# imazen/codec-eval

Measured on AMD Instinct MI355X. Metric: metric MP/s (SSIMULACRA2+DSSIM+Butteraugli) at 1/2/4/8 GPU; HBM-roofline %, higher is better.
Workload: dtype f32

## Files before the change

codec-eval_amd/csrc/dssim.hip:

```cpp
#include <algorithm>
#include <cstdlib>

#include "ce_internal.h"
#include "dssim_common.h"

namespace {

constexpr int TPB = 256;

__device__ __forceinline__ uint32_t slot_of(uint32_t z, uint32_t n_refs_used, uint32_t max_refs)
{
    return z < n_refs_used ? z : max_refs + (z - n_refs_used);
}

__global__ __launch_bounds__(TPB) void k_rgb8_to_rgba_f32(const uint8_t *__restrict__ rgb, const float *__restrict__ lut,
                                                          float4 *__restrict__ out, size_t n)
{
    __shared__ float s_lut[256];
    s_lut[threadIdx.x] = lut[threadIdx.x];
    __syncthreads();
    for (size_t i = (size_t)blockIdx.x * TPB + threadIdx.x; i < n; i += (size_t)gridDim.x * TPB)
        out[i] = make_float4(s_lut[rgb[3 * i]], s_lut[rgb[3 * i + 1]], s_lut[rgb[3 * i + 2]], 1.0f);
}

__device__ __forceinline__ double block_sum(double v, double *s_red)
{
#pragma unroll
    for (int off = 32; off > 0; off >>= 1) v += __shfl_down(v, off, 64);
    if ((threadIdx.x & 63) == 0) s_red[threadIdx.x >> 6] = v;
    __syncthreads();
    double t = 0.0;
    if (threadIdx.x == 0)
        for (int k = 0; k < TPB / 64; k++) t += s_red[k];
    __syncthreads();
    return t;
}

struct ds_tail {
    uint32_t w[CE_DSSIM_SCALES], h[CE_DSSIM_SCALES], pitch[CE_DSSIM_SCALES], n_part[CE_DSSIM_SCALES], gx[CE_DSSIM_SCALES];
    uint32_t blk_end[CE_DSSIM_SCALES];
    size_t plane[CE_DSSIM_SCALES], map_off[CE_DSSIM_SCALES];
};

__global__ __launch_bounds__(TPB) void k_dssim_avg(const double *__restrict__ part, double *__restrict__ avg_out, ds_tail t, uint32_t n_levels,
                                                   uint32_t n_blocks)
{
    __shared__ double s_red[TPB];
    const uint32_t p = blockIdx.x, level = blockIdx.y;
    const double *pp = part + ((size_t)p * n_levels + level) * 2 * n_blocks;
    const uint32_t used_blocks = t.n_part[level];
    double v = 0.0;
    for (uint32_t k = threadIdx.x; k < used_blocks; k += TPB) v += pp[k];
    s_red[threadIdx.x] = v;
    __syncthreads();
    for (int off = TPB / 2; off > 0; off >>= 1) {
        if ((int)threadIdx.x < off) s_red[threadIdx.x] += s_red[threadIdx.x + off];
        __syncthreads();
    }
    if (threadIdx.x == 0) {
        double avg = s_red[0] / (double)((size_t)t.w[level] * t.h[level]);
        if (!(avg > 0.0)) avg = 0.0;
        avg_out[(size_t)p * n_levels + level] = pow(avg, pow(0.5, (double)level));
    }
}

constexpr int AD_ROWS = 32;
__global__ __launch_bounds__(TPB) void k_dssim_absdev(const float *__restrict__ map, const double *__restrict__ avg_in,
                                                      double *__restrict__ part, ds_tail t, uint32_t n_levels, uint32_t n_blocks)
{
    __shared__ double s_red[TPB / 64];
    const uint32_t per_pair = t.blk_end[n_levels - 1], p = blockIdx.x / per_pair, bi = blockIdx.x % per_pair;
    uint32_t level = 0, first = 0;
#pragma unroll
    for (int l = 0; l + 1 < CE_DSSIM_SCALES; l++)
        if (l + 1 < (int)n_levels && bi >= t.blk_end[l]) level = l + 1, first = t.blk_end[l];
    const uint32_t w = t.w[level], h = t.h[level], pitch = t.pitch[level], gx = t.gx[level];
    const uint32_t bx = (bi - first) % gx, by = (bi - first) / gx;
    double *pp = part + ((size_t)p * n_levels + level) * 2 * n_blocks;
    const double avg = avg_in[(size_t)p * n_levels + level];
    const float *m = map + t.map_off[level] + (size_t)p * t.plane[level];
    const uint32_t x = bx * 64 + (threadIdx.x & 63);
    double val = 0.0;
#pragma unroll
    for (int k = 0; k < AD_ROWS / 4; k++) {
        const uint32_t y = by * AD_ROWS + 4 * k + (threadIdx.x >> 6);
        if (x < w && y < h) val += fabs(avg - (double)m[(size_t)y * pitch + x]);
    }
    const double s = block_sum(val, s_red);
    if (threadIdx.x == 0) pp[n_blocks + by * gx + bx] = s;
}

struct ds_geom {
    uint32_t npix[CE_DSSIM_SCALES];
    uint32_t nblk[CE_DSSIM_SCALES];
};

__global__ __launch_bounds__(64) void k_dssim_finalize_pairs(const double *__restrict__ part, double *__restrict__ level_scores,
                                                             ce_dev_scores *__restrict__ scores, uint32_t n_pairs,
                                                             uint32_t n_levels, uint32_t n_blocks, ds_geom g)
{
    const uint32_t p = blockIdx.x, lane = threadIdx.x;
    if (p >= n_pairs) return;
    const double W[CE_DSSIM_SCALES] = {0.028, 0.197, 0.322, 0.298, 0.155};
    double ssim_sum = 0.0, weight_sum = 0.0;
    for (uint32_t l = 0; l < n_levels; l++) {
        const double *pp = part + (((size_t)p * n_levels + l) * 2 + 1) * n_blocks;
        double dev = 0.0;
        for (uint32_t k = lane; k < g.nblk[l]; k += 64) dev += pp[k];
#pragma unroll
        for (int off = 32; off > 0; off >>= 1) dev += __shfl_down(dev, off, 64);
        dev = __shfl(dev, 0, 64);
        const double score = 1.0 - dev / (double)g.npix[l];
        if (lane == 0) level_scores[(size_t)p * CE_DSSIM_SCALES + l] = score;
        ssim_sum += score * W[l];
        weight_sum += W[l];
    }
    double ssim = ssim_sum / weight_sum;
    if (!(ssim > 2.220446049250313e-16)) ssim = 2.220446049250313e-16;
    if (lane == 0) scores[p].dssim = 1.0 / ssim - 1.0;
}

size_t map_offset(const ce_batch *b, int l)
{
    size_t off = 0;
    for (int k = 0; k < l; k++) off += (size_t)b->max_pairs * b->ds[k].plane;
    return off;
}

}

void ce_dssim_free(ce_batch *b)
{
    for (auto &p : b->ds_lin) hipFree(p), p = nullptr;
    hipFree(b->ds_img); hipFree(b->ds_map);
    for (int l = 0; l < CE_DSSIM_SCALES; l++) {
        hipFree(b->ds_rimg[l]); hipFree(b->ds_rmu[l]); hipFree(b->ds_rsq[l]);
        b->ds_rimg[l] = b->ds_rmu[l] = b->ds_rsq[l] = nullptr;
        ce_free_xcd_list(&b->ds_gwork[l]);
    }
    b->ds_ref_src = nullptr;
    hipFree(b->ds_part); hipFree(b->ds_level_scores); hipFree(b->ds_cells);
    b->ds_img = b->ds_map = b->ds_cells = nullptr;
    b->ds_cells_cap = 0;
    b->ds_map_pairs = 0;
    b->ds_part = b->ds_level_scores = nullptr;
    b->dssim_ready = false;
}

static int dssim_allocate(ce_batch *b)
{
    ce_ctx *ctx = b->ctx;
    uint32_t lw[CE_DSSIM_SCALES], lh[CE_DSSIM_SCALES];
    const int n = (int)ce_plan_dssim_levels(b->w, b->h, CE_DSSIM_SCALES, lw, lh);
    for (int l = 0; l < n; l++) {
        auto &d = b->ds[l];
        d.w = lw[l];
        d.h = lh[l];
        d.pitch = (d.w + 31u) & ~31u;
        d.plane = (size_t)d.pitch * d.h;
    }
    b->ds_levels = n;
    const size_t slots = (size_t)b->max_refs + b->max_pairs, p0 = b->ds[0].plane;
    const size_t p1 = n > 1 ? b->ds[1].plane : 1;
    CE_HIP(ctx, hipMalloc(&b->ds_lin[0], slots * 3 * p1 * sizeof(float)));
    CE_HIP(ctx, hipMalloc(&b->ds_lin[1], slots * 3 * p1 * sizeof(float)));
    CE_HIP(ctx, hipMalloc(&b->ds_img, (size_t)b->max_pairs * 3 * p0 * sizeof(float)));
    for (int l = 0; l < n; l++) {
        const size_t rb = (size_t)b->max_refs * 3 * b->ds[l].plane * sizeof(float);
        CE_HIP(ctx, hipMalloc(&b->ds_rimg[l], rb));
        CE_HIP(ctx, hipMalloc(&b->ds_rmu[l], rb));
        CE_HIP(ctx, hipMalloc(&b->ds_rsq[l], rb));
    }
    CE_HIP(ctx, hipMalloc(&b->ds_map, map_offset(b, n) * sizeof(float)));
    b->ds_blocks = std::max(((b->ds[0].w + 63) / 64) * ((b->ds[0].h + AD_ROWS - 1) / AD_ROWS), ((b->ds[0].w + CE_DSSIM_STRIP - 1) / CE_DSSIM_STRIP) * ((b->ds[0].h + 1) / 2));
    CE_HIP(ctx, hipMalloc(&b->ds_part, (size_t)b->max_pairs * CE_DSSIM_SCALES * 2 * b->ds_blocks * sizeof(double)));
    CE_HIP(ctx, hipMalloc(&b->ds_level_scores, (size_t)b->max_pairs * CE_DSSIM_SCALES * sizeof(double)));
    return CE_OK;
}

static int dssim_prepare(ce_batch *b)
{
    if (b->dssim_ready) return CE_OK;
    const int rc = dssim_allocate(b);
    if (rc != CE_OK) {
        const std::string why = b->ctx->err;
        ce_dssim_free(b);
        (void)hipGetLastError();
        b->ctx->err = why;
        return rc;
    }
    b->dssim_ready = true;
    return CE_OK;
}

int ce_launch_dssim(ce_batch *b, const uint8_t *d_refs, uint32_t n_refs_used, uint32_t n_pairs)
{
    ce_ctx *ctx = b->ctx;
    int rc = dssim_prepare(b);
    if (rc != CE_OK) return rc;
    const bool cached = b->keep_ref_pyramid && b->ds_ref_src == d_refs && b->ds_ref_count >= n_refs_used;
    const uint32_t z0 = cached ? n_refs_used : 0;
    if (!cached) b->ref_builds[1]++;
    ds_geom g{};
    ds_tail tail{};
    for (int l = 0; l < b->ds_levels; l++) {
        const auto &d = b->ds[l];
        if ((rc = ce_dssim_create_stream(b, l, d_refs, n_refs_used, n_pairs, z0)) != CE_OK) return rc;
        uint32_t n_part = 0;
        if ((rc = ce_dssim_compare_stream(b, l, n_pairs, b->ds_map + map_offset(b, l), &n_part)) != CE_OK) return rc;
        tail.w[l] = d.w, tail.h[l] = d.h, tail.pitch[l] = d.pitch, tail.plane[l] = d.plane, tail.n_part[l] = n_part;
        tail.gx[l] = (d.w + 63) / 64;
        tail.map_off[l] = map_offset(b, l);
        g.npix[l] = d.w * d.h;
        g.nblk[l] = tail.gx[l] * ((d.h + AD_ROWS - 1) / AD_ROWS);
        tail.blk_end[l] = (l ? tail.blk_end[l - 1] : 0u) + g.nblk[l];
    }
    {
        const uint32_t nl = (uint32_t)b->ds_levels;
        CE_LAUNCH(ctx, "dssim_avg", k_dssim_avg, dim3(n_pairs, nl), dim3(TPB), 0, b->ds_part, b->ds_level_scores, tail, nl, b->ds_blocks);
        const dim3 gp(tail.blk_end[nl - 1] * n_pairs);
        CE_LAUNCH(ctx, "dssim_absdev", k_dssim_absdev, gp, dim3(TPB), 0, (const float *)b->ds_map, b->ds_level_scores, b->ds_part, tail, nl,
                  b->ds_blocks);
    }
    if (b->keep_ref_pyramid && !cached) {
        b->ds_ref_src = d_refs;
        b->ds_ref_count = n_refs_used;
    }
    CE_LAUNCH(ctx, "dssim_finalize", k_dssim_finalize_pairs, dim3(n_pairs), dim3(64), 0, b->ds_part,
              b->ds_level_scores, b->d_scores, n_pairs, (uint32_t)b->ds_levels, b->ds_blocks, g);
    CE_HIP(ctx, hipGetLastError());
    return CE_OK;
}

int ce_dssim_read_maps(ce_batch *b, uint32_t level, uint32_t first, uint32_t count, uint32_t block, float *maps, double *ssim)
{
    ce_ctx *ctx = b->ctx;
    if (ssim) {
        CE_HIP(ctx, hipMemcpy2DAsync(ssim, sizeof(double), b->ds_level_scores + (size_t)first * CE_DSSIM_SCALES + level,
                                     CE_DSSIM_SCALES * sizeof(double), sizeof(double), count, hipMemcpyDeviceToHost, ctx->stream));
        if (!maps) CE_HIP(ctx, hipStreamSynchronize(ctx->stream));
    }
    if (!maps) return CE_OK;
    const auto &d = b->ds[level];
    return ce_read_map_cells(b, "dssim_block_min", b->ds_map + map_offset(b, (int)level), ce_map_geom{d.w, d.h, d.pitch, d.plane},
                             first, count, block, true, &b->ds_cells, &b->ds_cells_cap, maps);
}

int ce_launch_rgb8_to_dssim_image(ce_ctx *ctx, const uint8_t *d_rgb, float *d_rgba, size_t n_pixels)
{
    if (n_pixels == 0) return CE_OK;
    size_t blocks = std::min<size_t>((n_pixels + TPB - 1) / TPB, 4096);
    CE_LAUNCH(ctx, "rgb8_to_dssim_image", k_rgb8_to_rgba_f32, dim3((uint32_t)blocks), dim3(TPB), 0, d_rgb, ctx->d_lut_powf,
              reinterpret_cast<float4 *>(d_rgba), n_pixels);
    CE_HIP(ctx, hipGetLastError());
    return CE_OK;
}
```

codec-eval_amd/csrc/dssim_stream.hip:

```cpp
#include <algorithm>
#include <cstdlib>
#include <string>
#include <type_traits>

#include "ce_internal.h"
#include "dssim_common.h"

namespace {

constexpr int CS_OUT = CE_DSSIM_STRIP;
constexpr int CS_WAVES = 4;

__device__ __forceinline__ float lane_left(float v)
{
    return __builtin_bit_cast(float, __builtin_amdgcn_mov_dpp(__builtin_bit_cast(int, v), 0x138, 0xf, 0xf, true));
}
__device__ __forceinline__ float lane_right(float v)
{
    return __builtin_bit_cast(float, __builtin_amdgcn_mov_dpp(__builtin_bit_cast(int, v), 0x130, 0xf, 0xf, true));
}
__device__ __forceinline__ float ld_at(const float *base, uint32_t byte_off)
{
    return *reinterpret_cast<const float *>(reinterpret_cast<const char *>(base) + byte_off);
}

template <int N>
struct rowsN {
    float c[N], e[N], lr[N];
};
typedef rowsN<9> rows9;
struct rowin {
    float a[3], r[3];
};

template <int NP>
__device__ __forceinline__ float pass_rows(const rowsN<NP> &P, const rowsN<NP> &M, rowsN<NP> &N, int k, float v, float c_above)
{
    const float K0 = 0.095332f, K1 = 0.118095f, K4 = 0.146293f;
    const float corners = (P.lr[k] + lane_left(v)) + lane_right(v);
    const float edges = M.e[k] + v;
    N.c[k] = v;
    N.e[k] = (c_above + lane_left(v)) + lane_right(v);
    N.lr[k] = lane_left(v) + lane_right(v);
    return corners * K0 + edges * K1 + M.c[k] * K4;
}

struct cmp_planes {
    const float *t[3], *r[3], *u[3], *q[3];
};

template <bool EDGE>
__device__ __forceinline__ double dssim_compare_strip(const cmp_planes &pl, float *__restrict__ map, const lvl_geom &g, int xs, int y0, int y1)
{
    const int w = (int)g.w, h = (int)g.h, lane = (int)(threadIdx.x & 63);
    const uint32_t pitch = g.pitch;
    const int X = xs + lane - 2;
    const uint32_t Xc = (uint32_t)min(max(X, 0), w - 1);
    const bool out_lane = lane >= 2 && lane < 2 + CS_OUT && X < w;
    const bool before_first = X == -1, after_last = X == w;
    auto row_off = [&](int y) { return ((uint32_t)min(max(y, 0), h - 1) * pitch + Xc) * 4u; };
    double val = 0.0;
    auto step = [&](auto ends, const rows9 &P1, rows9 &M1, rows9 &N1, const rows9 &P2, rows9 &M2, rows9 &N2, const rowin &cur, rowin &nxt, int i)
                    __attribute__((always_inline)) {
        constexpr bool ENDS = decltype(ends)::value;
        const int t = i - 1, y = i - 2;
        float u1[3], q1[3];
        {
            const uint32_t o = row_off(i + 1), os = row_off(y);
#pragma unroll
            for (int c = 0; c < 3; c++) {
                nxt.a[c] = ld_at(pl.t[c], o);
                nxt.r[c] = ld_at(pl.r[c], o);
                u1[c] = ld_at(pl.u[c], os);
                q1[c] = ld_at(pl.q[c], os);
            }
        }
        float O[9];
#pragma unroll
        for (int c = 0; c < 3; c++) {
            const float v3[3] = {cur.a[c], cur.r[c] * cur.a[c], cur.a[c] * cur.a[c]};
#pragma unroll
            for (int j = 0; j < 3; j++) {
                const int k = 3 * c + j;
                float T = pass_rows(P1, M1, N1, k, v3[j], M1.c[k]);
                if (EDGE) {
                    const float fl = lane_right(T), fr = lane_left(T);
                    T = before_first ? fl : (after_last ? fr : T);
                }
                float c_above = M2.c[k];
                if (ENDS && t == h) T = M2.c[k];
                if (ENDS && t == 0) c_above = T;
                O[k] = pass_rows(P2, M2, N2, k, T, c_above);
                if (ENDS && t == 0) M2.lr[k] = N2.lr[k];
            }
            __builtin_amdgcn_sched_barrier(0);
        }
        if (y >= y0 && y < y1) {
            const float c1 = 0.01f * 0.01f, c2 = 0.03f * 0.03f, third = 1.0f / 3.0f;
            float m11[3], m12[3], m22[3], s1[3], s2[3], s12c[3];
#pragma unroll
            for (int c = 0; c < 3; c++) {
                const float u2v = O[3 * c + 0], s12 = O[3 * c + 1], q2 = O[3 * c + 2];
                m11[c] = u1[c] * u1[c];
                m12[c] = u1[c] * u2v;
                m22[c] = u2v * u2v;
                s1[c] = q1[c] - m11[c];
                s2[c] = q2 - m22[c];
                s12c[c] = s12 - m12[c];
            }
#define AVG3(v) (((v)[0] + (v)[1] + (v)[2]) * third)
            const float mu1_sq = AVG3(m11), mu2_sq = AVG3(m22), mu1_mu2 = AVG3(m12);
            const float sigma1_sq = AVG3(s1), sigma2_sq = AVG3(s2), sigma12 = AVG3(s12c);
#undef AVG3
            const float ssim = (2.0f * mu1_mu2 + c1) * (2.0f * sigma12 + c2) / ((mu1_sq + mu2_sq + c1) * (sigma1_sq + sigma2_sq + c2));
            if (out_lane) {
                map[(uint32_t)y * pitch + (uint32_t)X] = ssim;
                val += (double)ssim;
            }
        }
        __builtin_amdgcn_sched_barrier(0);
    };
    rows9 s0, s1, s2, z0, z1, z2;
#pragma unroll
    for (int k = 0; k < 9; k++) s0.lr[k] = s1.c[k] = s1.e[k] = s1.lr[k] = z0.lr[k] = z1.c[k] = z1.e[k] = z1.lr[k] = 0.f;
    rowin L0, L1, L2;
    const int i0 = y0 == 0 ? -1 : y0 - 2, n_bodies = (y1 + 1 - i0) / 3 + 1;
    {
        const uint32_t o = row_off(i0);
#pragma unroll
        for (int c = 0; c < 3; c++) L0.a[c] = ld_at(pl.t[c], o), L0.r[c] = ld_at(pl.r[c], o);
    }
    auto body = [&](auto ends, int i) __attribute__((always_inline)) {
        step(ends, s0, s1, s2, z0, z1, z2, L0, L1, i);
        step(ends, s1, s2, s0, z1, z2, z0, L1, L2, i + 1);
        step(ends, s2, s0, s1, z2, z0, z1, L2, L0, i + 2);
    };
    int i = i0;
    body(std::true_type{}, i);
    i += 3;
#pragma unroll 1
    for (int b = 1; b < n_bodies - 1; b++, i += 3) body(std::false_type{}, i);
    if (n_bodies > 1) body(std::true_type{}, i);
    return val;
}

__global__ __launch_bounds__(CS_WAVES * 64) __attribute__((amdgpu_waves_per_eu(3, 3))) void k_dssim_compare_stream(const float *__restrict__ img, const float *__restrict__ rimg,
                                                                        const float *__restrict__ rmu, const float *__restrict__ rsq,
                                                                        const uint32_t *__restrict__ pair_ref, float *__restrict__ map,
                                                                        double *__restrict__ part, lvl_geom g, uint32_t level,
                                                                        uint32_t n_levels, uint32_t n_blocks,
                                                                        const uint2 *__restrict__ work, uint32_t strips, uint32_t rows)
{
    const uint32_t wv = __builtin_amdgcn_readfirstlane(threadIdx.x >> 6);
    const uint2 wi = work[((blockIdx.x >> 3) * CS_WAVES + wv) * 8 + (blockIdx.x & 7)];
    const uint32_t tile = __builtin_amdgcn_readfirstlane(wi.x), p = __builtin_amdgcn_readfirstlane(wi.y);
    if (tile == ~0u) return;
    const uint32_t ref = __builtin_amdgcn_readfirstlane(pair_ref[p]);
    const int xs = (int)(tile % strips) * CS_OUT, y0 = (int)((tile / strips) * rows), y1 = min(y0 + (int)rows, (int)g.h);
    cmp_planes pl;
#pragma unroll
    for (int c = 0; c < 3; c++) {
        pl.t[c] = img + ((size_t)p * 3 + c) * g.plane;
        pl.r[c] = rimg + ((size_t)ref * 3 + c) * g.plane;
        pl.u[c] = rmu + ((size_t)ref * 3 + c) * g.plane;
        pl.q[c] = rsq + ((size_t)ref * 3 + c) * g.plane;
    }
    float *pmap = map + (size_t)p * g.plane;
    double val = (xs == 0 || xs + CS_OUT + 2 >= (int)g.w) ? dssim_compare_strip<true>(pl, pmap, g, xs, y0, y1)
                                                          : dssim_compare_strip<false>(pl, pmap, g, xs, y0, y1);
#pragma unroll
    for (int off = 32; off > 0; off >>= 1) val += __shfl_down(val, off, 64);
    if ((threadIdx.x & 63) == 0) part[(((size_t)p * n_levels + level) * 2 + 0) * n_blocks + tile] = val;
}

constexpr int CR_HALO_REF = 4, CR_HALO_DIST = 2;

template <int SRC, bool REF, bool EDGE>
__device__ __forceinline__ void dssim_create_strip(const uint8_t *__restrict__ src8, const float *const (&srcf)[3], const float *s_lut,
                                                   float *const (&lin_out)[3], float *const (&oimg)[3], float *const (&omu)[3],
                                                   float *const (&osq)[3], const lvl_geom &g, const lvl_geom &gn, int has_next, int xs,
                                                   int y0, int y1)
{
    constexpr bool FROM_U8 = SRC == CE_SRC_U8, FROM_U16 = SRC == CE_SRC_U16;
    constexpr int H = REF ? CR_HALO_REF : CR_HALO_DIST, OUT = 64 - 2 * H;
    const int w = (int)g.w, h = (int)g.h, lane = (int)(threadIdx.x & 63);
    const uint32_t pitch = g.pitch;
    const int X = xs + lane - H;
    const uint32_t Xc = (uint32_t)min(max(X, 0), w - 1);
    const bool out_lane = lane >= H && lane < H + OUT && X < w;
    const bool before_first = X == -1, after_last = X == w;
    auto edge_fix = [&](float T) {
        if (!EDGE) return T;
        const float fl = lane_right(T), fr = lane_left(T);
        return before_first ? fl : (after_last ? fr : T);
    };
    struct rgb { float v[3]; };
    struct raw3 { uint32_t v[3]; };
    auto request = [&](int y, raw3 &o) {
        const uint32_t yc = (uint32_t)min(max(y, 0), h - 1);
        if (FROM_U8) {
            const uint8_t *px = src8 + (yc * (uint32_t)w + Xc) * 3u;
            o.v[0] = px[0], o.v[1] = px[1], o.v[2] = px[2];
        } else if (FROM_U16) {
            const uint16_t *px = reinterpret_cast<const uint16_t *>(src8) + (yc * (uint32_t)w + Xc) * 3u;
            o.v[0] = px[0], o.v[1] = px[1], o.v[2] = px[2];
        } else if (SRC == CE_SRC_LIN) {
            const float *px = reinterpret_cast<const float *>(src8) + (yc * (uint32_t)w + Xc) * 3u;
#pragma unroll
            for (int c = 0; c < 3; c++) o.v[c] = __float_as_uint(px[c]);
        } else {
            const uint32_t ob = (yc * pitch + Xc) * 4u;
#pragma unroll
            for (int c = 0; c < 3; c++) o.v[c] = __float_as_uint(ld_at(srcf[c], ob));
        }
    };
    auto linear = [&](const raw3 &r, rgb &o) {
#pragma unroll
        for (int c = 0; c < 3; c++) o.v[c] = (FROM_U8 || FROM_U16) ? s_lut[r.v[c]] : __uint_as_float(r.v[c]);
    };
    constexpr int NS = REF ? 6 : 1;
    auto later_pass = [&](auto ends, auto &P, auto &M, auto &N, int k, float v, int r) __attribute__((always_inline)) {
        constexpr bool ENDS = decltype(ends)::value;
        float c_above = M.c[k];
        if (ENDS && r == h) v = M.c[k];
        if (ENDS && r == 0) c_above = v;
        const float o = pass_rows(P, M, N, k, v, c_above);
        if (ENDS && r == 0) M.lr[k] = N.lr[k];
        return o;
    };
    auto step = [&](auto ends, const rowsN<2> &Pa, rowsN<2> &Ma, rowsN<2> &Na, const rowsN<2> &Pb, rowsN<2> &Mb, rowsN<2> &Nb,
                    const rowsN<NS> &Pm, rowsN<NS> &Mm, rowsN<NS> &Nm, const rowsN<NS> &Pq, rowsN<NS> &Mq, rowsN<NS> &Nq,
                    const rgb &cur, rgb &nxt, const rgb &prev, const raw3 &arrived, raw3 &requested, float &L_new, const float &L_out,
                    int i) __attribute__((always_inline)) {
        request(i + 2, requested);
        linear(arrived, nxt);
        if (has_next && (i & 1) && i >= y0 && i < y1) {
            const int oy = i >> 1;
            float q[3];
#pragma unroll
            for (int c = 0; c < 3; c++) q[c] = (((prev.v[c] + lane_right(prev.v[c])) + cur.v[c]) + lane_right(cur.v[c])) * 0.25f;
            if (out_lane && !(X & 1) && (X >> 1) < (int)gn.w && oy < (int)gn.h) {
                const uint32_t o = (uint32_t)oy * gn.pitch + (uint32_t)(X >> 1);
#pragma unroll
                for (int c = 0; c < 3; c++) lin_out[c][o] = q[c];
            }
        }
        float L, A, B;
        rgb_to_lab(cur.v[0], cur.v[1], cur.v[2], L, A, B);
        L_new = L;
        const float ab[2] = {A, B};
        float img[3];
        img[0] = L_out;
#pragma unroll
        for (int k = 0; k < 2; k++) {
            const float T = edge_fix(pass_rows(Pa, Ma, Na, k, ab[k], Ma.c[k]));
            img[1 + k] = later_pass(ends, Pb, Mb, Nb, k, T, i - 1);
        }
        __builtin_amdgcn_sched_barrier(0);
        const int j = i - 2;
        if (j >= y0 && j < y1 && out_lane) {
            const uint32_t o = (uint32_t)j * pitch + (uint32_t)X;
#pragma unroll
            for (int c = 0; c < 3; c++) oimg[c][o] = img[c];
        }
        if (REF) {
            float O[6];
#pragma unroll
            for (int c = 0; c < 3; c++) {
                const float v = c == 0 ? img[0] : edge_fix(img[c]);
                const float two[2] = {v, v * v};
#pragma unroll
                for (int t = 0; t < 2; t++) {
                    const int k = 2 * c + t;
                    const float T = edge_fix(later_pass(ends, Pm, Mm, Nm, k, two[t], j));
                    O[k] = later_pass(ends, Pq, Mq, Nq, k, T, j - 1);
                }
                __builtin_amdgcn_sched_barrier(0);
            }
            const int y = i - 4;
            if (y >= y0 && y < y1 && out_lane) {
                const uint32_t o = (uint32_t)y * pitch + (uint32_t)X;
#pragma unroll
                for (int c = 0; c < 3; c++) omu[c][o] = O[2 * c], osq[c][o] = O[2 * c + 1];
            }
        }
    };
    rowsN<2> a0, a1, a2, b0, b1, b2;
    rowsN<NS> m0, m1, m2, q0, q1, q2;
#pragma unroll
    for (int k = 0; k < 2; k++) a0.lr[k] = a1.c[k] = a1.e[k] = a1.lr[k] = b0.lr[k] = b1.c[k] = b1.e[k] = b1.lr[k] = 0.f;
#pragma unroll
    for (int k = 0; k < NS; k++) m0.lr[k] = m1.c[k] = m1.e[k] = m1.lr[k] = q0.lr[k] = q1.c[k] = q1.e[k] = q1.lr[k] = 0.f;
    rgb R0, R1, R2;
    float l0 = 0.f, l1 = 0.f, l2 = 0.f;
    const int i0 = y0 == 0 ? -1 : y0 - H, i_last = y1 + H - 1, n_bodies = (i_last - i0) / 3 + 1;
    raw3 W0, W1, W2;
    request(i0, W2);
    request(i0 + 1, W0);
    linear(W2, R0);
    R2 = R0;
    auto body = [&](auto ends, int i) __attribute__((always_inline)) {
        step(ends, a0, a1, a2, b0, b1, b2, m0, m1, m2, q0, q1, q2, R0, R1, R2, W0, W1, l0, l1, i);
        step(ends, a1, a2, a0, b1, b2, b0, m1, m2, m0, q1, q2, q0, R1, R2, R0, W1, W2, l1, l2, i + 1);
        step(ends, a2, a0, a1, b2, b0, b1, m2, m0, m1, q2, q0, q1, R2, R0, R1, W2, W0, l2, l0, i + 2);
    };
    int i = i0, b = 0;
#pragma unroll 1
    for (; b < min(2, n_bodies); b++, i += 3) body(std::true_type{}, i);
#pragma unroll 1
    for (; b < n_bodies - 2; b++, i += 3) body(std::false_type{}, i);
#pragma unroll 1
    for (; b < n_bodies; b++, i += 3) body(std::true_type{}, i);
}

template <int SRC>
__global__ __launch_bounds__(CS_WAVES * 64) void k_dssim_create_stream(const uint8_t *__restrict__ refs, const uint8_t *__restrict__ tests,
                                                                       const float *__restrict__ lut, const float *__restrict__ lut_test,
                                                                       const float *__restrict__ lin_in,
                                                                       float *__restrict__ lin_out, float *__restrict__ img,
                                                                       float *__restrict__ rimg, float *__restrict__ rmu,
                                                                       float *__restrict__ rsq, lvl_geom g, lvl_geom gn, int has_next,
                                                                       size_t img_bytes, uint32_t n_refs_used, uint32_t max_refs, uint32_t z0,
                                                                       uint32_t rows)
{
    constexpr bool FROM_U8 = SRC == CE_SRC_U8, FROM_U16 = SRC == CE_SRC_U16;
    __shared__ float s_lut[256];
    if (FROM_U8) {
        s_lut[threadIdx.x] = lut[threadIdx.x];
        __syncthreads();
    }
    const uint32_t wv = __builtin_amdgcn_readfirstlane(threadIdx.x >> 6);
    const uint32_t z = blockIdx.y + z0;
    const bool is_ref = z < n_refs_used;
    const uint32_t slot = is_ref ? z : max_refs + (z - n_refs_used), oslot = is_ref ? z : z - n_refs_used;
    const uint32_t out_cols = 64 - 2 * (is_ref ? CR_HALO_REF : CR_HALO_DIST), strips = (g.w + out_cols - 1) / out_cols;
    const uint32_t tile = blockIdx.x * CS_WAVES + wv;
    if (tile >= strips * ((g.h + rows - 1) / rows)) return;
    const int xs = (int)((tile % strips) * out_cols), y0 = (int)((tile / strips) * rows), y1 = min(y0 + (int)rows, (int)g.h);
    const uint8_t *src8 = (FROM_U8 || FROM_U16 || SRC == CE_SRC_LIN) ? (is_ref ? refs + (size_t)z * img_bytes : tests + (size_t)(z - n_refs_used) * img_bytes) : nullptr;
    const float *srcf[3];
    float *lo[3], *oi[3], *om[3], *oq[3];
#pragma unroll
    for (int c = 0; c < 3; c++) {
        srcf[c] = lin_in + ((size_t)slot * 3 + c) * g.plane;
        lo[c] = lin_out + ((size_t)slot * 3 + c) * gn.plane;
        oi[c] = (is_ref ? rimg : img) + ((size_t)oslot * 3 + c) * g.plane;
        om[c] = rmu + ((size_t)oslot * 3 + c) * g.plane;
        oq[c] = rsq + ((size_t)oslot * 3 + c) * g.plane;
    }
    const float *tab = FROM_U16 ? (is_ref ? lut : lut_test) : s_lut;
    const bool edge = xs == 0 || xs + (int)out_cols + (is_ref ? CR_HALO_REF : CR_HALO_DIST) >= (int)g.w;
    if (is_ref) {
        if (edge)
            dssim_create_strip<SRC, true, true>(src8, srcf, tab, lo, oi, om, oq, g, gn, has_next, xs, y0, y1);
        else
            dssim_create_strip<SRC, true, false>(src8, srcf, tab, lo, oi, om, oq, g, gn, has_next, xs, y0, y1);
    } else {
        if (edge)
            dssim_create_strip<SRC, false, true>(src8, srcf, tab, lo, oi, om, oq, g, gn, has_next, xs, y0, y1);
        else
            dssim_create_strip<SRC, false, false>(src8, srcf, tab, lo, oi, om, oq, g, gn, has_next, xs, y0, y1);
    }
}

uint32_t stream_rows(uint32_t strips, uint32_t h, uint32_t n_images)
{
    static const size_t min_waves = [] {
        const char *e = std::getenv("CE_STREAM_MIN_WAVES");
        return e ? (size_t)std::atol(e) : (size_t)8192;
    }();
    uint32_t rows = 64;
    while (rows > 8 && (size_t)strips * ((h + rows - 1) / rows) * n_images < min_waves) rows /= 2;
    while (rows > 2 && (size_t)strips * ((h + rows - 1) / rows) * n_images < 1024) rows /= 2;
    return rows;
}

}

int ce_dssim_create_stream(ce_batch *b, int l, const uint8_t *d_refs, uint32_t n_refs_used, uint32_t n_pairs, uint32_t z0)
{
    ce_ctx *ctx = b->ctx;
    const auto &d = b->ds[l];
    const bool has_next = l + 1 < b->ds_levels;
    const auto &nd = b->ds[has_next ? l + 1 : l];
    const lvl_geom lg{d.w, d.h, d.pitch, d.plane}, ng{nd.w, nd.h, nd.pitch, nd.plane};
    const uint32_t n_slots = n_refs_used + n_pairs;
    if (n_slots <= z0) return CE_OK;
    const uint32_t strips_ref = (d.w + 64 - 2 * CR_HALO_REF - 1) / (64 - 2 * CR_HALO_REF), strips = (d.w + CS_OUT - 1) / CS_OUT;
    const uint32_t rows = b->debug_ds_rows ? b->debug_ds_rows : stream_rows(strips, d.h, n_slots - z0);
    const uint32_t tiles = std::max(z0 < n_refs_used ? strips_ref : 0u, strips) * ((d.h + rows - 1) / rows);
#define CE_CREATE_LAUNCH(NAME, U8, GRID, Z0, LUT_R, LUT_T)                                                                                      \
    CE_LAUNCH(ctx, NAME, (k_dssim_create_stream<U8>), GRID, dim3(CS_WAVES * 64), 0, d_refs, (const uint8_t *)b->d_tests,            \
              (const float *)LUT_R, (const float *)LUT_T, (const float *)(l == 0 ? nullptr : b->ds_lin[l & 1]), b->ds_lin[(l + 1) & 1], b->ds_img,      \
              b->ds_rimg[l], b->ds_rmu[l], b->ds_rsq[l], lg, ng, has_next ? 1 : 0, b->img_bytes, n_refs_used, b->max_refs, Z0, rows)
    const dim3 grid((tiles + CS_WAVES - 1) / CS_WAVES, n_slots - z0);
    if (l == 0 && b->linear) CE_CREATE_LAUNCH("dssim_create_lin", CE_SRC_LIN, grid, z0, nullptr, nullptr);
    else if (l == 0 && b->depth[0]) CE_CREATE_LAUNCH("dssim_create_u16", CE_SRC_U16, grid, z0, b->deep_lut[1][0], b->deep_lut[1][1]);
    else if (l == 0) CE_CREATE_LAUNCH("dssim_create_u8", CE_SRC_U8, grid, z0, ctx->d_lut_powf, ctx->d_lut_powf);
    else CE_CREATE_LAUNCH("dssim_create", CE_SRC_F32, grid, z0, ctx->d_lut_powf, ctx->d_lut_powf);
#undef CE_CREATE_LAUNCH
    return CE_OK;
}

int ce_dssim_compare_stream(ce_batch *b, int l, uint32_t n_pairs, float *level_map, uint32_t *n_part)
{
    ce_ctx *ctx = b->ctx;
    const auto &d = b->ds[l];
    const lvl_geom lg{d.w, d.h, d.pitch, d.plane};
    const uint32_t strips = (d.w + CS_OUT - 1) / CS_OUT, rows = b->debug_ds_rows ? b->debug_ds_rows : stream_rows(strips, d.h, n_pairs);
    const int rc = ce_build_xcd_list(b, n_pairs, ce_xcd_keys{1, (d.h + rows - 1) / rows, strips, CS_WAVES}, &b->ds_gwork[l]);
    if (rc != CE_OK) return rc;
    CE_LAUNCH(ctx, "dssim_compare", k_dssim_compare_stream, dim3(b->ds_gwork[l].len / CS_WAVES), dim3(CS_WAVES * 64), 0,
              (const float *)b->ds_img, (const float *)b->ds_rimg[l], (const float *)b->ds_rmu[l], (const float *)b->ds_rsq[l],
              b->d_pair_ref, level_map, b->ds_part, lg, (uint32_t)l, (uint32_t)b->ds_levels, b->ds_blocks,
              (const uint2 *)b->ds_gwork[l].d, strips, rows);
    *n_part = strips * ((d.h + rows - 1) / rows);
    return CE_OK;
}
```

Before: 19100.

## Batch DSSIM absdev rows per block and use bpermute for edge reflection

The absdev kernel now has each block cover several consecutive 32-row tiles, prefetching the next tile's map values while it reduces the current one. This cuts the number of blocks launched and overlaps load latency with the reduction. In the streaming compare and create kernels, the two DPP moves plus selects used for edge mirroring become a single ds_bpermute with a per-lane source index. The pass_rows shuffles are hoisted, and an asm barrier pins the evaluation order of the sums. bpermute goes through the LDS crossbar, so it may add latency compared with DPP. The extra per-block serial loop also reduces parallelism on the smaller pyramid levels.

Measured after the change: 19320 (median of 6 runs). 1.01x the previous value.

```diff
diff --git a/codec-eval_amd/csrc/dssim.hip b/codec-eval_amd/csrc/dssim.hip
--- a/codec-eval_amd/csrc/dssim.hip
+++ b/codec-eval_amd/csrc/dssim.hip
@@ -65,6 +65,7 @@
 }
 
 constexpr int AD_ROWS = 32;
+constexpr int AD_SUB = 4;
 __global__ __launch_bounds__(TPB) void k_dssim_absdev(const float *__restrict__ map, const double *__restrict__ avg_in,
                                                       double *__restrict__ part, ds_tail t, uint32_t n_levels, uint32_t n_blocks)
 {
@@ -75,19 +76,35 @@
     for (int l = 0; l + 1 < CE_DSSIM_SCALES; l++)
         if (l + 1 < (int)n_levels && bi >= t.blk_end[l]) level = l + 1, first = t.blk_end[l];
     const uint32_t w = t.w[level], h = t.h[level], pitch = t.pitch[level], gx = t.gx[level];
-    const uint32_t bx = (bi - first) % gx, by = (bi - first) / gx;
+    const uint32_t bx = (bi - first) % gx, by0 = (bi - first) / gx * AD_SUB, by1 = min(by0 + AD_SUB, (h + AD_ROWS - 1) / AD_ROWS);
     double *pp = part + ((size_t)p * n_levels + level) * 2 * n_blocks;
     const double avg = avg_in[(size_t)p * n_levels + level];
     const float *m = map + t.map_off[level] + (size_t)p * t.plane[level];
     const uint32_t x = bx * 64 + (threadIdx.x & 63);
-    double val = 0.0;
-#pragma unroll
-    for (int k = 0; k < AD_ROWS / 4; k++) {
-        const uint32_t y = by * AD_ROWS + 4 * k + (threadIdx.x >> 6);
-        if (x < w && y < h) val += fabs(avg - (double)m[(size_t)y * pitch + x]);
-    }
-    const double s = block_sum(val, s_red);
-    if (threadIdx.x == 0) pp[n_blocks + by * gx + bx] = s;
+    float v[AD_ROWS / 4], nv[AD_ROWS / 4];
+    auto load = [&](uint32_t by, float (&o)[AD_ROWS / 4]) {
+#pragma unroll
+        for (int k = 0; k < AD_ROWS / 4; k++) {
+            const uint32_t y = by * AD_ROWS + 4 * k + (threadIdx.x >> 6);
+            o[k] = (x < w && y < h) ? m[(size_t)y * pitch + x] : 0.f;
+        }
+    };
+    load(by0, v);
+    for (uint32_t by = by0; by < by1; by++) {
+        if (by + 1 < by1) load(by + 1, nv);
+        double val = 0.0;
+#pragma unroll
+        for (int k = 0; k < AD_ROWS / 4; k++) {
+            const uint32_t y = by * AD_ROWS + 4 * k + (threadIdx.x >> 6);
+            if (x < w && y < h) val += fabs(avg - (double)v[k]);
+        }
+        const double s = block_sum(val, s_red);
+        if (threadIdx.x == 0) pp[n_blocks + by * gx + bx] = s;
+        if (by + 1 < by1) {
+#pragma unroll
+            for (int k = 0; k < AD_ROWS / 4; k++) v[k] = nv[k];
+        }
+    }
 }
 
 struct ds_geom {
@@ -213,7 +230,7 @@
         tail.map_off[l] = map_offset(b, l);
         g.npix[l] = d.w * d.h;
         g.nblk[l] = tail.gx[l] * ((d.h + AD_ROWS - 1) / AD_ROWS);
-        tail.blk_end[l] = (l ? tail.blk_end[l - 1] : 0u) + g.nblk[l];
+        tail.blk_end[l] = (l ? tail.blk_end[l - 1] : 0u) + tail.gx[l] * (((d.h + AD_ROWS - 1) / AD_ROWS + AD_SUB - 1) / AD_SUB);
     }
     {
         const uint32_t nl = (uint32_t)b->ds_levels;
diff --git a/codec-eval_amd/csrc/dssim_stream.hip b/codec-eval_amd/csrc/dssim_stream.hip
--- a/codec-eval_amd/csrc/dssim_stream.hip
+++ b/codec-eval_amd/csrc/dssim_stream.hip
@@ -18,6 +18,10 @@
 __device__ __forceinline__ float lane_right(float v)
 {
     return __builtin_bit_cast(float, __builtin_amdgcn_mov_dpp(__builtin_bit_cast(int, v), 0x130, 0xf, 0xf, true));
+}
+__device__ __forceinline__ float lane_from(float v, int src_lane_x4)
+{
+    return __builtin_bit_cast(float, __builtin_amdgcn_ds_bpermute(src_lane_x4, __builtin_bit_cast(int, v)));
 }
 __device__ __forceinline__ float ld_at(const float *base, uint32_t byte_off)
 {
@@ -37,11 +41,14 @@
 __device__ __forceinline__ float pass_rows(const rowsN<NP> &P, const rowsN<NP> &M, rowsN<NP> &N, int k, float v, float c_above)
 {
     const float K0 = 0.095332f, K1 = 0.118095f, K4 = 0.146293f;
-    const float corners = (P.lr[k] + lane_left(v)) + lane_right(v);
+    const float l = lane_left(v), r = lane_right(v);
+    float corners = (P.lr[k] + l) + r;
+    float e = (c_above + l) + r, lr = l + r;
+    asm("" : "+v"(corners), "+v"(e), "+v"(lr));
     const float edges = M.e[k] + v;
     N.c[k] = v;
-    N.e[k] = (c_above + lane_left(v)) + lane_right(v);
-    N.lr[k] = lane_left(v) + lane_right(v);
+    N.e[k] = e;
+    N.lr[k] = lr;
     return corners * K0 + edges * K1 + M.c[k] * K4;
 }
 
@@ -57,7 +64,7 @@
     const int X = xs + lane - 2;
     const uint32_t Xc = (uint32_t)min(max(X, 0), w - 1);
     const bool out_lane = lane >= 2 && lane < 2 + CS_OUT && X < w;
-    const bool before_first = X == -1, after_last = X == w;
+    const int edge_src = (lane + (X == -1 ? 1 : (X == w ? -1 : 0))) * 4;
     auto row_off = [&](int y) { return ((uint32_t)min(max(y, 0), h - 1) * pitch + Xc) * 4u; };
     double val = 0.0;
     auto step = [&](auto ends, const rows9 &P1, rows9 &M1, rows9 &N1, const rows9 &P2, rows9 &M2, rows9 &N2, const rowin &cur, rowin &nxt, int i)
@@ -79,14 +86,17 @@
 #pragma unroll
         for (int c = 0; c < 3; c++) {
             const float v3[3] = {cur.a[c], cur.r[c] * cur.a[c], cur.a[c] * cur.a[c]};
+            float T3[3];
 #pragma unroll
             for (int j = 0; j < 3; j++) {
                 const int k = 3 * c + j;
-                float T = pass_rows(P1, M1, N1, k, v3[j], M1.c[k]);
-                if (EDGE) {
-                    const float fl = lane_right(T), fr = lane_left(T);
-                    T = before_first ? fl : (after_last ? fr : T);
-                }
+                T3[j] = pass_rows(P1, M1, N1, k, v3[j], M1.c[k]);
+                if (EDGE) T3[j] = lane_from(T3[j], edge_src);
+            }
+#pragma unroll
+            for (int j = 0; j < 3; j++) {
+                const int k = 3 * c + j;
+                float T = T3[j];
                 float c_above = M2.c[k];
                 if (ENDS && t == h) T = M2.c[k];
                 if (ENDS && t == 0) c_above = T;
@@ -188,11 +198,9 @@
     const int X = xs + lane - H;
     const uint32_t Xc = (uint32_t)min(max(X, 0), w - 1);
     const bool out_lane = lane >= H && lane < H + OUT && X < w;
-    const bool before_first = X == -1, after_last = X == w;
+    const int edge_src = (lane + (X == -1 ? 1 : (X == w ? -1 : 0))) * 4;
     auto edge_fix = [&](float T) {
-        if (!EDGE) return T;
-        const float fl = lane_right(T), fr = lane_left(T);
-        return before_first ? fl : (after_last ? fr : T);
+        return EDGE ? lane_from(T, edge_src) : T;
     };
     struct rgb { float v[3]; };
     struct raw3 { uint32_t v[3]; };
```
